# seanrjohnson/protein_gibbs_sampler

Hardware: AMD Instinct MI355X
Metric: sampled positions/sec (whole node), ESM-1b L=256 B=256 Gibbs (higher is better)
Workload: dtype bf16

## Files before the change

include/pgibbs.h:

```cpp
#ifndef PGIBBS_H
#define PGIBBS_H

#include <stdint.h>

#ifdef __cplusplus
extern "C" {
#endif

#define PG_OK 0
#define PG_ERR_INVALID 1
#define PG_ERR_HIP 2
#define PG_ERR_NO_DEVICE 3
#define PG_ERR_WEIGHTS 4
#define PG_ERR_UNSUPPORTED 5
#define PG_ERR_RANGE 6

const char* pg_version(void);
const char* pg_last_error(void);
int pg_device_count(void);

typedef struct pg_pyrandom pg_pyrandom;
pg_pyrandom* pg_pyrandom_create(void);
void pg_pyrandom_destroy(pg_pyrandom*);
int pg_pyrandom_seed(pg_pyrandom*, const uint32_t* key_words, int n_words);
// ... 104 lines not shown
                     int32_t* d_out);
typedef int (*pg_allgather_fn)(void* ctx, const void* send, void* recv, size_t n_int32);
int pg_dbg_gather_tokens_host(int rank, int world, const int32_t* local, int64_t rows, int width, const int64_t* counts,
                              int force_padded, pg_allgather_fn allgather, void* ctx, int32_t* out);
int pg_dbg_gather_plan(int rank, int world, int64_t rows, int width, const int64_t* counts, int force_padded, int64_t* out7,
                       int64_t* out_off_bytes);

int pg_prof_enable(pg_engine*, int on);
int pg_prof_reset(pg_engine*);
int pg_prof_get(pg_engine*, const char* kernel_class, double* total_ms, int64_t* launches);
int pg_prof_get_kernels(pg_engine*, const char* kernel_class, char* buf, int buf_bytes);

int pg_dbg_gemm(int device, int precision, const float* x, const float* w, const float* bias, float* out, int M, int N,
                int K, int epi);
int pg_dbg_gemm_bench(int device, int M, int N, int K, int epi, int variant, int iters, double* avg_ms);
int pg_dbg_gemm_plan(int M, int N, int K, int epi, int variant, int have_ws, int m_live, int n_cu, char* buf, int buf_bytes);
int pg_dbg_rowln_bench(int device, int M, int K, int iters, double* ms, double* max_diff);
int pg_dbg_qkv_attention_bench(int device, int B, int T, int H, int iters, double* ms, double* max_diff);
int pg_dbg_layernorm(int device, const float* x, const float* gamma, const float* beta, float* y, int M, int d,
                     float eps);
int pg_dbg_layernorm_operand(int device, int precision, const float* x, const float* gamma, const float* beta, float* y, int M,
                             int d, float eps);
int pg_dbg_attention(int device, int precision, const float* qkv, float* ctx, int B, int T, int H);
int pg_dbg_rope(int device, int precision, float* qkv_inout, int B, int T, int H);

int pg_dbg_msa_attention(int device, int which, const float* qkv, float* ctx, int B, int R, int C, int H, float scale);

#ifdef __cplusplus
}
#endif
#endif
```

protein_gibbs_sampler_amd/_lib.py:

```python
import ctypes
import math
import os
import sys
from ctypes import (POINTER, Structure, c_char_p, c_double, c_float, c_int, c_int32, c_int64, c_uint32, c_uint64,
                    c_void_p)

_HERE = os.path.dirname(os.path.abspath(__file__))
LIB_PATH = os.environ.get("PGIBBS_LIB_PATH") or os.path.join(_HERE, "lib", "libpgibbs.so")

PG_OK = 0
PG_ERR_INVALID, PG_ERR_HIP, PG_ERR_NO_DEVICE, PG_ERR_WEIGHTS, PG_ERR_UNSUPPORTED, PG_ERR_RANGE = 1, 2, 3, 4, 5, 6
PG_ARCH_ESM1B, PG_ARCH_MSA1B, PG_ARCH_ESM1, PG_ARCH_ESM2 = 1, 2, 3, 4
PG_COMM_ID_BYTES = 128
PG_PREC_BF16, PG_PREC_FP32, PG_PREC_F16 = 0, 1, 2
INT32_MAX = 2**31 - 1


class PgError(RuntimeError):
    def __init__(self, code, msg):
        super().__init__("pgibbs error %d: %s" % (code, msg))
        self.code = code
        self.msg = msg


# ... 63 lines not shown
    ("pg_mask_scatter_device", c_int, [c_void_p, c_void_p, c_int64, c_int, c_void_p, c_void_p, c_int64, c_int, c_int]),
    ("pg_sample_writeback_device", c_int, [c_void_p, c_void_p, c_int64, c_int, c_void_p, c_int, c_void_p, c_void_p, c_int64,
                                           c_int, POINTER(SampleParams), c_int, c_void_p]),
    ("pg_comm_unique_id", c_int, [c_void_p]),
    ("pg_comm_create", c_int, [c_int, c_int, c_void_p, c_int, POINTER(c_void_p)]),
    ("pg_comm_destroy", None, [c_void_p]),
    ("pg_comm_rank", c_int, [c_void_p]),
    ("pg_comm_world", c_int, [c_void_p]),
    ("pg_gather_tokens", c_int, [c_void_p, c_void_p, c_void_p, c_int64, c_int, POINTER(c_int64), c_void_p]),
    ("pg_dbg_gather_tokens_host", c_int, [c_int, c_int, c_void_p, c_int64, c_int, POINTER(c_int64), c_int, c_void_p, c_void_p, c_void_p]),
    ("pg_dbg_gather_plan", c_int, [c_int, c_int, c_int64, c_int, POINTER(c_int64), c_int, POINTER(c_int64), POINTER(c_int64)]),
    ("pg_prof_enable", c_int, [c_void_p, c_int]),
    ("pg_prof_reset", c_int, [c_void_p]),
    ("pg_prof_get", c_int, [c_void_p, c_char_p, POINTER(c_double), POINTER(c_int64)]),
    ("pg_prof_get_kernels", c_int, [c_void_p, c_char_p, c_char_p, c_int]),
    ("pg_dbg_gemm", c_int, [c_int, c_int, c_void_p, c_void_p, c_void_p, c_void_p, c_int, c_int, c_int, c_int]),
    ("pg_dbg_gemm_bench", c_int, [c_int, c_int, c_int, c_int, c_int, c_int, c_int, POINTER(c_double)]),
    ("pg_dbg_gemm_plan", c_int, [c_int, c_int, c_int, c_int, c_int, c_int, c_int, c_int, c_char_p, c_int]),
    ("pg_dbg_rowln_bench", c_int, [c_int, c_int, c_int, c_int, POINTER(c_double), POINTER(c_double)]),
    ("pg_dbg_qkv_attention_bench", c_int, [c_int, c_int, c_int, c_int, c_int, POINTER(c_double), POINTER(c_double)]),
    ("pg_dbg_layernorm", c_int, [c_int, c_void_p, c_void_p, c_void_p, c_void_p, c_int, c_int, c_float]),
    ("pg_dbg_layernorm_operand", c_int, [c_int, c_int, c_void_p, c_void_p, c_void_p, c_void_p, c_int, c_int, c_float]),
    ("pg_dbg_attention", c_int, [c_int, c_int, c_void_p, c_void_p, c_int, c_int, c_int]),
    ("pg_dbg_rope", c_int, [c_int, c_int, c_void_p, c_int, c_int, c_int]),
    ("pg_dbg_msa_attention", c_int, [c_int, c_int, c_void_p, c_void_p, c_int, c_int, c_int, c_int, c_float]),
]


def lib():
    global _lib
    if _lib is not None:
        return _lib
    if not os.path.exists(LIB_PATH):
        raise ImportError(
            "protein_gibbs_sampler_amd: the HIP library %s is missing. Build it with "
            "`python -c 'import __graft_entry__ as g; g.build()'` (or `make -C protein_gibbs_sampler_amd/csrc`). "
            "There is no CPU fallback." % LIB_PATH)
    if os.environ.get("PGIBBS_HIP_RUNTIME", "auto") != "system":
        try:
            import torch
        except ImportError:
            pass
    handle = ctypes.CDLL(LIB_PATH, mode=ctypes.RTLD_GLOBAL)
    for name, restype, argtypes in SIGNATURES:
        fn = getattr(handle, name)
        fn.restype = restype
# ... 34 lines not shown
```

protein_gibbs_sampler_amd/csrc/api.hip:

```cpp
#include <math.h>
#include <string.h>

#include <vector>

#include <algorithm>

#include "engine.h"
#include "gemm_epilogue.h"

namespace pg {
const char* last_error_cstr();
}
using namespace pg;

namespace {
struct DeviceGuard {
  int prev = -1;
  explicit DeviceGuard(int dev) {
    (void)hipGetDevice(&prev);
    if (dev >= 0 && dev != prev) (void)hipSetDevice(dev);
  }
  ~DeviceGuard() {
    if (prev >= 0) (void)hipSetDevice(prev);
  }
// ... 747 lines not shown
  Tmp t;
  float* dq = (float*)t.get((size_t)M * 3 * d * 4);
  if (precision == PG_PREC_FP32) {
    bf16_t* c3 = (bf16_t*)t.get((size_t)M * 3 * d * 2);
    if (!dq || !c3) return fail(PG_ERR_HIP, "hipMalloc failed");
    PG_HIP(hipMemcpy(dq, qkv, (size_t)M * 3 * d * 4, hipMemcpyHostToDevice));
    const SeqLayout chain = {1, T, 0, 1};
    if ((rc = launch_attention_f32(nullptr, dq, c3, d, B, T, H, 3 * d, 3 * d, d, 2 * d, chain))) return rc;
    return split3_rows_to_host(c3, ctx, M, d);
  }
  bf16_t* bq = (bf16_t*)t.get((size_t)M * 3 * d * 2);
  bf16_t* bc = (bf16_t*)t.get((size_t)M * d * 2);
  float* dc = (float*)t.get((size_t)M * d * 4);
  if (!dq || !bq || !bc || !dc) return fail(PG_ERR_HIP, "hipMalloc failed");
  PG_HIP(hipMemcpy(dq, qkv, (size_t)M * 3 * d * 4, hipMemcpyHostToDevice));
  if ((rc = OPS(launch_f32_to_bf16, nullptr, dq, bq, M * 3 * d, 1.f))) return rc;
  if ((rc = OPS(launch_attention_bf16, nullptr, bq, bc, B, T, H, 3 * d, d, d, 2 * d, nullptr, -1))) return rc;
  if ((rc = OPS(launch_bf16_to_f32, nullptr, bc, dc, M * d))) return rc;
  PG_HIP(hipDeviceSynchronize());
  PG_HIP(hipMemcpy(ctx, dc, (size_t)M * d * 4, hipMemcpyDeviceToHost));
  return PG_OK;
}

int pg_dbg_layernorm_operand(int device, int precision, const float* x, const float* gamma, const float* beta, float* y, int M, int d,
                             float eps) {
  if (precision != PG_PREC_BF16 && precision != PG_PREC_FP32 && precision != PG_PREC_F16) return fail(PG_ERR_INVALID, "unknown precision mode");
  if (!x || !gamma || !beta || !y || M < 1 || d < 32 || d % 32) return fail(PG_ERR_INVALID, "pg_dbg_layernorm_operand: bad argument");
  DeviceGuard g(-1);
  int rc = dbg_device(device);
  if (rc) return rc;
  const bool split = precision == PG_PREC_FP32;
  Tmp t;
  float* dx = (float*)t.get((size_t)M * d * 4);
  float* dg = (float*)t.get((size_t)d * 4);
  float* dbt = (float*)t.get((size_t)d * 4);
  float* dy = (float*)t.get((size_t)M * d * 4);
  bf16_t* h = (bf16_t*)t.get((size_t)M * d * 2 * (split ? 3 : 1));
  if (!dx || !dg || !dbt || !dy || !h) return fail(PG_ERR_HIP, "hipMalloc failed");
  PG_HIP(hipMemcpy(dx, x, (size_t)M * d * 4, hipMemcpyHostToDevice));
  PG_HIP(hipMemcpy(dg, gamma, (size_t)d * 4, hipMemcpyHostToDevice));
  PG_HIP(hipMemcpy(dbt, beta, (size_t)d * 4, hipMemcpyHostToDevice));
  if ((rc = OPS(launch_layernorm_bf16, nullptr, dx, dg, dbt, h, M, d, eps, split, 0, 0, true))) return rc;
  if (split) return split3_rows_to_host(h, y, M, d);
  if ((rc = OPS(launch_bf16_to_f32, nullptr, h, dy, (int64_t)M * d))) return rc;
  PG_HIP(hipDeviceSynchronize());
  PG_HIP(hipMemcpy(y, dy, (size_t)M * d * 4, hipMemcpyDeviceToHost));
// ... 75 lines not shown
```

protein_gibbs_sampler_amd/csrc/attention.hip:

```cpp
#include <stdlib.h>

#include "kernels.h"

PG_OPS_BEGIN

typedef __attribute__((ext_vector_type(8))) __bf16 bf16x8;
typedef __attribute__((ext_vector_type(4))) float f32x4;
typedef __attribute__((ext_vector_type(2))) float f32x2;

typedef short v4s __attribute__((ext_vector_type(4)));

#ifdef PG_ATT_PROF
__device__ unsigned long long* pg_att_prof;
#define PG_T(slot, i)                                                                                              \
  do {                                                                                                             \
    if ((slot) < 8 && (threadIdx.x & 63) == 0)                                                                     \
      pg_att_prof[(((size_t)blockIdx.x * 4 + (threadIdx.x >> 6)) * 8 + (slot)) * 8 + (i)] = __builtin_readcyclecounter(); \
  } while (0)
#else
#define PG_T(slot, i)
#endif

template <int MAXKB, bool PADMASK, bool BIASKV = false, bool SPLIT = false>
__global__ __launch_bounds__(256, (MAXKB <= 18 ? 2 : 1)) void attention_kernel(const bf16_t* __restrict__ qkv, bf16_t* __restrict__ ctx, int T,
                                                       int H, int ld_qkv_, int ld_ctx_, int k_off, int v_off,
                                                       SeqLayout sl, const int32_t* __restrict__ key_tok, int pad_idx,
                                                       const bf16_t* __restrict__ bias_kv, int split_from = 0, int split = 1) {
  __shared__ __attribute__((aligned(16))) char smem[2 * MAXKB * 16 * 128 + (PADMASK ? MAXKB * 16 : 0)];
  char* Ks = smem;
  char* Vs = smem + MAXKB * 16 * 128;
  char* padf = smem + 2 * MAXKB * 16 * 128;

  const int tid = threadIdx.x, lane = tid & 63, wave = tid >> 6;
  PG_T(7, 0);
  int pair = blockIdx.x, qb_first = wave, qb_step = 4;
  if (SPLIT && (int)blockIdx.x >= split_from) {
    const int u = blockIdx.x - split_from;
    pair = split_from + u / split;
    qb_first = u % split + split * wave;
    qb_step = 4 * split;
  }
  const int seq = pair / H, h = pair % H;
  const size_t row0 = (size_t)(seq / sl.inner_count) * sl.outer_rows + (size_t)(seq % sl.inner_count) * sl.inner_rows;
  const size_t ld_qkv = (size_t)ld_qkv_ * sl.row_step, ld_ctx = (size_t)ld_ctx_ * sl.row_step;
  const bf16_t* base = qkv + row0 * ld_qkv_ + h * 64;
  const int Tk = T + (BIASKV ? 1 : 0);
  constexpr int nkc = MAXKB / 2;
  constexpr int tpad = MAXKB * 16;

  {
    constexpr int NIT = (MAXKB * 16 * 8 + 255) / 256;
    uint4 kreg[NIT], vreg[NIT];
#pragma unroll
    for (int it = 0; it < NIT; ++it) {
      const int i = tid + it * 256;
      const int row = i >> 3, c = i & 7;
      kreg[it] = make_uint4(0, 0, 0, 0);
      vreg[it] = make_uint4(0, 0, 0, 0);
      if (i < tpad * 8 && row < T) {
        kreg[it] = *(const uint4*)(base + (size_t)row * ld_qkv + k_off + c * 8);
        vreg[it] = *(const uint4*)(base + (size_t)row * ld_qkv + v_off + c * 8);
      } else if (BIASKV && row == T) {
        kreg[it] = *(const uint4*)(bias_kv + h * 64 + c * 8);
        vreg[it] = *(const uint4*)(bias_kv + (H + h) * 64 + c * 8);
      }
    }
#pragma unroll
    for (int it = 0; it < NIT; ++it) {
      const int i = tid + it * 256;
      if (i < tpad * 8) {
// ... 3 lines not shown
      }
    }
  }
  if (PADMASK) {
    for (int key = tid; key < MAXKB * 16; key += 256)
      padf[key] = (key < T && key_tok[row0 + (size_t)key * sl.row_step] == pad_idx) ? 1 : 0;
  }
  PG_T(7, 1);
  __syncthreads();
  PG_T(7, 2);

  const int fr = lane & 15, fq = lane >> 4;
  const int nqb = (T + 15) >> 4;
  bf16x8 qf[2], qn[2];
  auto load_q = [&](int qb, bf16x8 (&dst)[2]) {
    int qrow = qb * 16 + fr;
    if (qrow >= T) qrow = T - 1;
#pragma unroll
    for (int kk = 0; kk < 2; ++kk) dst[kk] = *(const bf16x8*)(base + (size_t)qrow * ld_qkv + kk * 32 + fq * 8);
  };
  if (qb_first < nqb) load_q(qb_first, qf);
  for (int qb = qb_first; qb < nqb; qb += qb_step) {
    if (qb + qb_step < nqb) load_q(qb + qb_step, qn);
    PG_T(qb >> 2, 0);

    f32x4 st[MAXKB];
    {
      constexpr int CH = (MAXKB % 6 == 0) ? 6 : (MAXKB % 4 == 0 ? 4 : 2);
      bf16x8 kbuf[2][CH][2];
      auto load_chunk = [&](int ch, bf16x8 (&dst)[CH][2]) {
#pragma unroll
        for (int u = 0; u < CH; ++u) {
#if defined(PG_ATT_PROF) && PG_ATT_ABL == 1
          const int krow = (ch * CH + (u > 0 ? 0 : u)) * 16 + fr;
          if (u > 0) { dst[u][0] = dst[0][0]; dst[u][1] = dst[0][1]; continue; }
#else
          const int krow = (ch * CH + u) * 16 + fr;
#endif
#pragma unroll
          for (int kk = 0; kk < 2; ++kk) dst[u][kk] = *(const bf16x8*)(Ks + krow * 128 + (((kk * 4 + fq) ^ (krow & 7)) << 4));
        }
      };
      load_chunk(0, kbuf[0]);
#pragma unroll
      for (int ch = 0; ch < MAXKB / CH; ++ch) {
        if (ch + 1 < MAXKB / CH) load_chunk(ch + 1, kbuf[(ch + 1) & 1]);
        __builtin_amdgcn_sched_barrier(0);
#pragma unroll
        for (int u = 0; u < CH; ++u)
          st[ch * CH + u] = mfma_op16(kbuf[ch & 1][u][0], qf[0], (f32x4){0.f, 0.f, 0.f, 0.f});
#pragma unroll
        for (int u = 0; u < CH; ++u)
          st[ch * CH + u] = mfma_op16(kbuf[ch & 1][u][1], qf[1], st[ch * CH + u]);
        __builtin_amdgcn_sched_barrier(0);
      }
    }
    PG_T(qb >> 2, 1);
    float mx = -3.0e38f;
    int tl = Tk - fq * 4;
    asm volatile("" : "+v"(tl));
#pragma unroll
    for (int kb = MAXKB > 6 ? MAXKB - 6 : 0; kb < MAXKB; ++kb)
      if ((kb + 1) * 16 > Tk) {
#pragma unroll
        for (int r = 0; r < 4; ++r)
          if (kb * 16 + r >= tl) st[kb][r] = -3.0e38f;
      }
#pragma unroll
    for (int kb = 0; kb < MAXKB; ++kb)
#pragma unroll
      for (int r = 0; r < 4; ++r) mx = fmaxf(mx, st[kb][r]);
    if (PADMASK) {
      const float fill = sl.row_step == 1 ? -3.0e38f : -10000.0f;
      mx = -3.0e38f;
#pragma unroll
      for (int kb = 0; kb < MAXKB; ++kb) {
        const uint32_t f4 = *(const uint32_t*)(padf + kb * 16 + fq * 4);
#pragma unroll
        for (int r = 0; r < 4; ++r) {
          if ((f4 >> (8 * r)) & 0xffu) st[kb][r] = fill;
          mx = fmaxf(mx, st[kb][r]);
        }
      }
    }
    mx = rows4_max(mx);
    const f32x2 l2e = {1.44269504088896341f, 1.44269504088896341f};
    const float mneg1 = -mx * 1.44269504088896341f;
    const f32x2 mneg = {mneg1, mneg1};
    f32x2 sum2 = {0.f, 0.f};
#pragma unroll
    for (int kb = 0; kb < MAXKB; ++kb) {
      const f32x2 a = __builtin_elementwise_fma((f32x2){st[kb][0], st[kb][1]}, l2e, mneg);
      const f32x2 b = __builtin_elementwise_fma((f32x2){st[kb][2], st[kb][3]}, l2e, mneg);
      const f32x2 ea = {__builtin_amdgcn_exp2f(a[0]), __builtin_amdgcn_exp2f(a[1])};
      const f32x2 eb = {__builtin_amdgcn_exp2f(b[0]), __builtin_amdgcn_exp2f(b[1])};
      st[kb] = (f32x4){ea[0], ea[1], eb[0], eb[1]};
      sum2 += ea;
      sum2 += eb;
    }
    float sum = sum2[0] + sum2[1];
    sum = rows4_sum(sum);
    const float inv = 1.0f / sum;
    PG_T(qb >> 2, 2);

    f32x4 o[4];
#pragma unroll
    for (int db = 0; db < 4; ++db) o[db] = (f32x4){0.f, 0.f, 0.f, 0.f};
    {
      union VF { bf16x8 v; uint2 h[2]; };
      VF vbuf[3][4];
      auto load_v = [&](int c, VF (&dst)[4]) {
#pragma unroll
        for (int db = 0; db < 4; ++db) {
#if defined(PG_ATT_PROF) && PG_ATT_ABL == 2
          if (db > 0) { dst[db] = dst[0]; continue; }
#endif
#pragma unroll
          for (int hh = 0; hh < 2; ++hh) {
            const int krow = (2 * c + hh) * 16 + fq * 4 + (fr >> 2);
            const int dcol = db * 16 + (fr & 3) * 4;
            const char* a = Vs + krow * 128 + (((dcol >> 3) ^ (krow & 7)) << 4) + ((dcol >> 2) & 1) * 8;
            const v4s t = __builtin_amdgcn_ds_read_tr16_b64_v4i16((v4s __attribute__((address_space(3)))*)(
                (__attribute__((address_space(3))) char*)a));
            dst[db].h[hh] = __builtin_bit_cast(uint2, t);
          }
        }
      };
      load_v(0, vbuf[0]);
      if (nkc > 1) load_v(1, vbuf[1]);
#pragma unroll
      for (int c = 0; c < nkc; ++c) {
        if (c + 2 < nkc) load_v(c + 2, vbuf[(c + 2) % 3]);
        union { bf16x8 v; uint32_t u[4]; } pf;
        const f32x4 lo = st[2 * c], hi = st[2 * c + 1];
        pf.u[0] = pack_op2(lo[0], lo[1]);
        pf.u[1] = pack_op2(lo[2], lo[3]);
        pf.u[2] = pack_op2(hi[0], hi[1]);
        pf.u[3] = pack_op2(hi[2], hi[3]);
        __builtin_amdgcn_sched_barrier(0);
#pragma unroll
        for (int db = 0; db < 4; ++db) o[db] = mfma_op16(vbuf[c % 3][db].v, pf.v, o[db]);
        __builtin_amdgcn_sched_barrier(0);
      }
    }
    PG_T(qb >> 2, 3);
    const int q = qb * 16 + fr;
    if (q < T) {
      bf16_t* dst = ctx + row0 * ld_ctx_ + (size_t)q * ld_ctx + h * 64 + fq * 4;
#pragma unroll
      for (int db = 0; db < 4; ++db) {
        uint2 p;
        p.x = pack_op2(o[db][0] * inv, o[db][1] * inv);
        p.y = pack_op2(o[db][2] * inv, o[db][3] * inv);
        *(uint2*)(dst + db * 16) = p;
      }
    }
    qf[0] = qn[0];
    qf[1] = qn[1];
    PG_T(qb >> 2, 4);
  }
  PG_T(7, 3);
}

template <int MAXKB, int OCC, bool PADMASK, bool BIASKV>
__global__ __launch_bounds__(256, OCC) void attention_long_kernel(const bf16_t* __restrict__ qkv, bf16_t* __restrict__ ctx, int T,
                                                               int H, int ld_qkv_, int ld_ctx_, int k_off, int v_off,
                                                               SeqLayout sl, int n_qchunk, const int32_t* __restrict__ key_tok_,
                                                               int pad_idx, const bf16_t* __restrict__ bias_kv_) {
  const int32_t* __restrict__ key_tok = PADMASK ? key_tok_ : nullptr;
  const bf16_t* __restrict__ bias_kv = BIASKV ? bias_kv_ : nullptr;
  constexpr int tpad = MAXKB * 16, nkc = MAXKB / 2;
  __shared__ __attribute__((aligned(16))) char smem[2 * tpad * 128 + (PADMASK ? tpad : 0)];
  char* Ks = smem;
  char* Vs = smem + tpad * 128;
  char* padf = smem + 2 * tpad * 128;
  const int tid = threadIdx.x, lane = tid & 63, wave = tid >> 6;
  const int qc = blockIdx.x % n_qchunk, sh = blockIdx.x / n_qchunk;
  const int seq = sh / H, h = sh % H;
  const size_t row0 = (size_t)(seq / sl.inner_count) * sl.outer_rows + (size_t)(seq % sl.inner_count) * sl.inner_rows;
  const size_t ld_qkv = (size_t)ld_qkv_ * sl.row_step, ld_ctx = (size_t)ld_ctx_ * sl.row_step;
  const bf16_t* base = qkv + row0 * ld_qkv_ + h * 64;
  const int fr = lane & 15, fq = lane >> 4;
  const int q0 = qc * 64 + wave * 16;
  const bool active = q0 < T;
// ... 120 lines not shown
      }
    }
  }
  const int q = q0 + fr;
  if (active && q < T) {
    const float inv = 1.0f / l;
    bf16_t* dst = ctx + row0 * ld_ctx_ + (size_t)q * ld_ctx + h * 64 + fq * 4;
#pragma unroll
    for (int db = 0; db < 4; ++db) {
      uint2 p;
      p.x = pack_op2(o[db][0] * inv, o[db][1] * inv);
      p.y = pack_op2(o[db][2] * inv, o[db][3] * inv);
      *(uint2*)(dst + db * 16) = p;
    }
  }
}

int launch_attention_bf16(hipStream_t s, const bf16_t* qkv, bf16_t* ctx, int B, int T, int H, int ld_qkv, int ld_ctx,
                          int k_off, int v_off, const int32_t* key_tok, int pad_idx, const bf16_t* bias_kv) {
  SeqLayout sl = {1, T, 0, 1};
  return launch_attention_seq_bf16(s, qkv, ctx, B, T, H, ld_qkv, ld_ctx, k_off, v_off, sl, key_tok, pad_idx, bias_kv);
}

int launch_attention_seq_bf16(hipStream_t s, const bf16_t* qkv, bf16_t* ctx, int64_t n_seq, int T, int H, int ld_qkv,
                              int ld_ctx, int k_off, int v_off, SeqLayout sl, const int32_t* key_tok, int pad_idx,
                              const bf16_t* bias_kv) {
  if (n_seq == 0) return 0;
  if (n_seq * H > 0x7fffffff) return fail(1, "attention: too many sequences");
  dim3 grid((unsigned)(n_seq * H)), block(256);
  static const int split_on = env_int("PGIBBS_ATTN_SPLIT", 1);
  const int n_cu = device_cu_count();
  int split_from = 0, split = 1;
  if (split_on && !key_tok && !bias_kv && sl.row_step == 1 && T >= 64 && T <= 576) {
    const int kb = (((T + 15) / 16) + 1) & ~1;
    const long pairs = n_seq * H, slots = (long)n_cu * (kb <= 20 ? 2 : 1);
    const long rem = pairs % slots;
    const int nqb = (T + 15) / 16;
    int sp = rem ? (int)(slots / rem) : 1;
    if (sp > 4) sp = 4;
    if (sp > nqb / 4) sp = nqb / 4;
    if (sp >= 2) {
      split = sp;
      split_from = (int)(pairs - rem);
      grid = dim3((unsigned)(split_from + rem * sp));
    }
  }
#define PG_ATT_SPLIT_LAUNCH(KB) hipLaunchKernelGGL((attention_kernel<KB, false, false, true>), grid, block, 0, s, qkv, ctx, T, H, ld_qkv, ld_ctx, k_off, v_off, sl, key_tok, pad_idx, bias_kv, split_from, split)
#define PG_ATT(KB)                                                                                             \
  else if (Tk <= KB * 16) {                                                                                    \
    if (bias_kv && key_tok) hipLaunchKernelGGL((attention_kernel<KB, true, true>), grid, block, 0, s, qkv, ctx, T, H, ld_qkv, ld_ctx, k_off, v_off, sl, key_tok, pad_idx, bias_kv); \
    else if (bias_kv) hipLaunchKernelGGL((attention_kernel<KB, false, true>), grid, block, 0, s, qkv, ctx, T, H, ld_qkv, ld_ctx, k_off, v_off, sl, key_tok, pad_idx, bias_kv); \
    else if (key_tok) hipLaunchKernelGGL((attention_kernel<KB, true>), grid, block, 0, s, qkv, ctx, T, H, ld_qkv, ld_ctx, k_off, v_off, sl, key_tok, pad_idx, bias_kv); \
    else if (split > 1) PG_ATT_SPLIT_LAUNCH(KB);                                                               \
    else hipLaunchKernelGGL((attention_kernel<KB, false>), grid, block, 0, s, qkv, ctx, T, H, ld_qkv, ld_ctx, k_off, v_off, sl, key_tok, pad_idx, bias_kv); \
  }
  const int Tk = T + (bias_kv ? 1 : 0);
  static const int fine_ladder = env_int("PGIBBS_ATTN_LADDER", 1);
  if (T <= 0) return fail(1, "attention: empty sequence");
#define PG_ATT_PLAIN(KB)                                                                                       \
  else if (fine_ladder && !bias_kv && Tk <= KB * 16) {                                                         \
    if (key_tok) hipLaunchKernelGGL((attention_kernel<KB, true>), grid, block, 0, s, qkv, ctx, T, H, ld_qkv, ld_ctx, k_off, v_off, sl, key_tok, pad_idx, bias_kv); \
    else if (split > 1) PG_ATT_SPLIT_LAUNCH(KB);                                                               \
    else hipLaunchKernelGGL((attention_kernel<KB, false>), grid, block, 0, s, qkv, ctx, T, H, ld_qkv, ld_ctx, k_off, v_off, sl, key_tok, pad_idx, bias_kv); \
  }
  PG_ATT(2) PG_ATT(4) PG_ATT_PLAIN(6) PG_ATT(8) PG_ATT_PLAIN(10) PG_ATT(12) PG_ATT_PLAIN(14) PG_ATT_PLAIN(16) PG_ATT(18)
  PG_ATT_PLAIN(20) PG_ATT_PLAIN(22) PG_ATT(24) PG_ATT_PLAIN(26) PG_ATT_PLAIN(28) PG_ATT(30) PG_ATT_PLAIN(32) PG_ATT_PLAIN(34) PG_ATT(36)
#undef PG_ATT_PLAIN
#undef PG_ATT
#undef PG_ATT_SPLIT_LAUNCH
  else {
    const int n_qchunk = (T + 63) / 64;
    if (n_seq * H * n_qchunk > 0x7fffffff) return fail(1, "attention: too many sequences");
    const dim3 g((unsigned)(n_seq * H * n_qchunk));
#define PG_ATT_LONG(P, B) hipLaunchKernelGGL((attention_long_kernel<18, 2, P, B>), g, block, 0, s, qkv, ctx, T, H, ld_qkv, ld_ctx, k_off, v_off, sl, n_qchunk, key_tok, pad_idx, bias_kv)
    if (key_tok && bias_kv) PG_ATT_LONG(true, true);
    else if (key_tok) PG_ATT_LONG(true, false);
    else if (bias_kv) PG_ATT_LONG(false, true);
    else PG_ATT_LONG(false, false);
#undef PG_ATT_LONG
  }
  PG_HIP(hipGetLastError());
  return 0;
}

PG_OPS_END
```

protein_gibbs_sampler_amd/csrc/kernels_ops.inc:

```
int launch_gemm_bf16(hipStream_t s, const bf16_t* X, const bf16_t* W, const float* bias, void* out, int M, int N, int K,
                     int ldx, int ldw, int ldo, int epi, float* ws = nullptr, size_t ws_bytes = 0, int m_live = 0);
int gemm_splitk_splits(int K);
size_t gemm_splitk_ws_bytes(int M, int N, int K);
int launch_gemm_bf16_variant(hipStream_t s, const bf16_t* X, const bf16_t* W, const float* bias, void* out, int M, int N,
                             int K, int ldx, int ldw, int ldo, int epi, int variant, float* ws = nullptr, size_t ws_bytes = 0,
                             int m_live = 0);

bool gemm_ln_skinny_ok(int M, int N, int K);
int launch_gemm_ln_skinny(hipStream_t s, const float* X, int ldx, const float* gamma, const float* beta, float eps, const bf16_t* W,
                          const float* bias, void* out, int M, int N, int K, int ldw, int ldo, int epi);
bool chain_trunk_ok(int M, int d_model, int d_ffn, int n_heads);
size_t chain_trunk_sync_bytes();
size_t chain_trunk_part_bytes(int M, int d_model);
int launch_chain_trunk(hipStream_t s, const PgChainTrunkArgs& a, int M, int d_model);
int launch_gemm_big(hipStream_t s, const bf16_t* X, const bf16_t* W, const float* bias, void* out, int M, int N, int K, int ldx,
                    int ldw, int ldo, int epi, int m_live = 0);
bool gemm_ladder_has(int epi, int h);
int launch_gemm_ladder(hipStream_t s, const bf16_t* X, const bf16_t* W, const float* bias, void* out, int m_live, int m_rows, int h,
                       int N, int K, int ldx, int ldw, int ldo, int epi);
bool gemm_rowln_ok(int m_rows, int N, int K);
int launch_gemm_rowln(hipStream_t s, const bf16_t* A, const bf16_t* W, const float* bias, float* x, const float* gamma,
                      const float* beta, bf16_t* h, int m_live, int m_rows, int K, int lda, int ldw, float eps, int colmajor_R = 0,
                      int colmajor_C = 0, int abl = 0);
void gemm_plan_text(int M, int N, int K, int epi, int variant, bool have_ws, int m_live, int n_cu, std::string* text);
void gemm_big_geometry(int M, int N, int K, int* m_main_panels, int* tail_rows);
int launch_gemm_w16(hipStream_t s, const bf16_t* X, const bf16_t* W, const float* bias, void* out, int M, int N, int K, int ldx,
                    int ldw, int ldo, int epi, int abl = 0, int tail_rows = 0);
int launch_gemm_split3(hipStream_t s, const bf16_t* X3, const bf16_t* W3, const float* bias, void* out, int M, int N, int K, int ldo,
                       int epi);
bool gemm_split3_fused(int M, int N, int K, int epi);
int launch_gemm_split3_w16(hipStream_t s, const bf16_t* X3, const bf16_t* W3, const float* bias, void* out, int M, int N, int K,
                           int ldo, int epi);

int launch_attention_bf16(hipStream_t s, const bf16_t* qkv, bf16_t* ctx, int B, int T, int H, int ld_qkv, int ld_ctx,
                          int k_off, int v_off, const int32_t* key_tok = nullptr, int pad_idx = -1, const bf16_t* bias_kv = nullptr);
int launch_attention_seq_bf16(hipStream_t s, const bf16_t* qkv, bf16_t* ctx, int64_t n_seq, int T, int H, int ld_qkv,
                              int ld_ctx, int k_off, int v_off, SeqLayout sl, const int32_t* key_tok = nullptr,
                              int pad_idx = -1, const bf16_t* bias_kv = nullptr);
size_t msa_row_split_scratch_bytes(int B, int R, int C, int H, int order_bh);
int launch_msa_row_attention_bf16(hipStream_t s, const bf16_t* qkv, bf16_t* ctx, int B, int R, int C, int H, int ld_qkv,
                                  int ld_ctx, int k_off, int v_off, float scale, float* partial = nullptr,
                                  size_t partial_bytes = 0, int order_bh = 0);

int launch_embed_ln(hipStream_t s, const int32_t* tokens, const float* embed, const float* pos, const float* msa_pos,
                    const float* gamma, const float* beta, float* x, int64_t n_tok, int T, int d, int pad_idx,
                    int mask_idx, int token_dropout, int rows_per_msa, float eps,
                    const float* gamma2 = nullptr, const float* beta2 = nullptr, bf16_t* h2 = nullptr,
                    float embed_scale = 1.0f);
int launch_rope(hipStream_t s, void* qkv, bool f32, const float* table, int table_rows, int64_t M, int T, int H, int ld);
int launch_layernorm_bf16(hipStream_t s, const float* x, const float* gamma, const float* beta, bf16_t* h, int64_t M,
                          int d, float eps, bool split3 = false,
                          int colmajor_R = 0, int colmajor_C = 0,
                          bool split3_dup = true);
bool colattn_ok(int R, int d_model, int n_heads);
int launch_gemm_colattn(hipStream_t s, const bf16_t* X, const bf16_t* W, const float* bias, bf16_t* ctx, int B, int R, int C, int H,
                        int d, int ld_ctx);
int launch_headmajor_qkv(hipStream_t s, const bf16_t* w, const float* b, bf16_t* w2, float* b2, int H, int K);
int launch_layernorm_f32(hipStream_t s, const float* x, const float* gamma, const float* beta, float* y, int64_t M, int d,
                         float eps);
int launch_gather_ln_bf16(hipStream_t s, const float* x, const int32_t* idx, const int32_t* row_map, int P, int width,
                          const float* gamma, const float* beta, bf16_t* h, int64_t n_sel, int d, float eps,
// ... 19 lines not shown
```

Measured before the change: 72600.

## Add persistent attention kernel with double-buffered K/V DMA and ticketed q-blocks

```diff
diff --git a/include/pgibbs.h b/include/pgibbs.h
--- a/include/pgibbs.h
+++ b/include/pgibbs.h
@@ -150,6 +150,8 @@
 int pg_dbg_layernorm_operand(int device, int precision, const float* x, const float* gamma, const float* beta, float* y, int M,
                              int d, float eps);
 int pg_dbg_attention(int device, int precision, const float* qkv, float* ctx, int B, int T, int H);
+int pg_dbg_attention_forms(int device, int precision, const uint16_t* qkv, uint16_t* ctx_plain, uint16_t* ctx_persistent, int B, int T,
+                           int H, int iters, double* ms);
 int pg_dbg_rope(int device, int precision, float* qkv_inout, int B, int T, int H);
 
 int pg_dbg_msa_attention(int device, int which, const float* qkv, float* ctx, int B, int R, int C, int H, float scale);
diff --git a/protein_gibbs_sampler_amd/_lib.py b/protein_gibbs_sampler_amd/_lib.py
--- a/protein_gibbs_sampler_amd/_lib.py
+++ b/protein_gibbs_sampler_amd/_lib.py
@@ -109,6 +109,7 @@
     ("pg_dbg_layernorm", c_int, [c_int, c_void_p, c_void_p, c_void_p, c_void_p, c_int, c_int, c_float]),
     ("pg_dbg_layernorm_operand", c_int, [c_int, c_int, c_void_p, c_void_p, c_void_p, c_void_p, c_int, c_int, c_float]),
     ("pg_dbg_attention", c_int, [c_int, c_int, c_void_p, c_void_p, c_int, c_int, c_int]),
+    ("pg_dbg_attention_forms", c_int, [c_int, c_int, c_void_p, c_void_p, c_void_p, c_int, c_int, c_int, c_int, POINTER(c_double)]),
     ("pg_dbg_rope", c_int, [c_int, c_int, c_void_p, c_int, c_int, c_int]),
     ("pg_dbg_msa_attention", c_int, [c_int, c_int, c_void_p, c_void_p, c_int, c_int, c_int, c_int, c_float]),
 ]
diff --git a/protein_gibbs_sampler_amd/csrc/api.hip b/protein_gibbs_sampler_amd/csrc/api.hip
--- a/protein_gibbs_sampler_amd/csrc/api.hip
+++ b/protein_gibbs_sampler_amd/csrc/api.hip
@@ -793,6 +793,47 @@
   return PG_OK;
 }
 
+int pg_dbg_attention_forms(int device, int precision, const uint16_t* qkv, uint16_t* ctx_plain, uint16_t* ctx_persistent, int B, int T,
+                           int H, int iters, double* ms) {
+  if (precision != PG_PREC_BF16 && precision != PG_PREC_F16) return fail(PG_ERR_INVALID, "pg_dbg_attention_forms: bf16 or fp16 operands");
+  if (!qkv || !ctx_plain || !ctx_persistent || B < 1 || T < 1 || H < 1 || (iters > 0 && !ms))
+    return fail(PG_ERR_INVALID, "pg_dbg_attention_forms: bad argument");
+  DeviceGuard g(-1);
+  int rc = dbg_device(device);
+  if (rc) return rc;
+  const int d = H * 64;
+  const size_t M = (size_t)B * T;
+  Tmp t;
+  bf16_t* bq = (bf16_t*)t.get(M * 3 * d * 2);
+  bf16_t* bc = (bf16_t*)t.get(M * d * 2);
+  if (!bq || !bc) return fail(PG_ERR_HIP, "hipMalloc failed");
+  PG_HIP(hipMemcpy(bq, qkv, M * 3 * d * 2, hipMemcpyHostToDevice));
+  const SeqLayout chain = {1, T, 0, 1};
+  hipEvent_t e0, e1;
+  PG_HIP(hipEventCreate(&e0));
+  PG_HIP(hipEventCreate(&e1));
+  for (int form = 1; form <= 2 && !rc; ++form) {
+    PG_HIP(hipMemset(bc, 0xff, M * d * 2));
+    rc = OPS(launch_attention_seq_bf16, nullptr, bq, bc, B, T, H, 3 * d, d, d, 2 * d, chain, nullptr, -1, nullptr, form);
+    if (rc) break;
+    PG_HIP(hipDeviceSynchronize());
+    PG_HIP(hipMemcpy(form == 1 ? ctx_plain : ctx_persistent, bc, M * d * 2, hipMemcpyDeviceToHost));
+    if (iters > 0) {
+      PG_HIP(hipEventRecord(e0, nullptr));
+      for (int it = 0; it < iters && !rc; ++it)
+        rc = OPS(launch_attention_seq_bf16, nullptr, bq, bc, B, T, H, 3 * d, d, d, 2 * d, chain, nullptr, -1, nullptr, form);
+      PG_HIP(hipEventRecord(e1, nullptr));
+      PG_HIP(hipEventSynchronize(e1));
+      float el = 0.f;
+      PG_HIP(hipEventElapsedTime(&el, e0, e1));
+      ms[form - 1] = el / iters;
+    }
+  }
+  (void)hipEventDestroy(e0);
+  (void)hipEventDestroy(e1);
+  return rc;
+}
+
 int pg_dbg_layernorm_operand(int device, int precision, const float* x, const float* gamma, const float* beta, float* y, int M, int d,
                              float eps) {
   if (precision != PG_PREC_BF16 && precision != PG_PREC_FP32 && precision != PG_PREC_F16) return fail(PG_ERR_INVALID, "unknown precision mode");
diff --git a/protein_gibbs_sampler_amd/csrc/attention.hip b/protein_gibbs_sampler_amd/csrc/attention.hip
--- a/protein_gibbs_sampler_amd/csrc/attention.hip
+++ b/protein_gibbs_sampler_amd/csrc/attention.hip
@@ -1,11 +1,10 @@
 #include <stdlib.h>
 
+#include "gemm_epilogue.h"
 #include "kernels.h"
 
 PG_OPS_BEGIN
 
-typedef __attribute__((ext_vector_type(8))) __bf16 bf16x8;
-typedef __attribute__((ext_vector_type(4))) float f32x4;
 typedef __attribute__((ext_vector_type(2))) float f32x2;
 
 typedef short v4s __attribute__((ext_vector_type(4)));
@@ -21,6 +20,146 @@
 #define PG_T(slot, i)
 #endif
 
+template <int MAXKB, bool PADMASK>
+__device__ __forceinline__ void attention_qblock(const char* Ks, const char* Vs, const char* padf, const bf16x8 (&qf)[2], int qb, int T,
+                                                 int Tk, float pad_fill, bf16_t* ctx_head, size_t ld_ctx, int fr, int fq, int slot) {
+  constexpr int nkc = MAXKB / 2;
+  PG_T(slot, 0);
+
+  f32x4 st[MAXKB];
+  {
+    constexpr int CH = (MAXKB % 6 == 0) ? 6 : (MAXKB % 4 == 0 ? 4 : 2);
+    bf16x8 kbuf[2][CH][2];
+    auto load_chunk = [&](int ch, bf16x8 (&dst)[CH][2]) {
+#pragma unroll
+      for (int u = 0; u < CH; ++u) {
+#if defined(PG_ATT_PROF) && PG_ATT_ABL == 1
+        const int krow = (ch * CH + (u > 0 ? 0 : u)) * 16 + fr;
+        if (u > 0) { dst[u][0] = dst[0][0]; dst[u][1] = dst[0][1]; continue; }
+#else
+        const int krow = (ch * CH + u) * 16 + fr;
+#endif
+#pragma unroll
+        for (int kk = 0; kk < 2; ++kk) dst[u][kk] = *(const bf16x8*)(Ks + krow * 128 + (((kk * 4 + fq) ^ (krow & 7)) << 4));
+      }
+    };
+    load_chunk(0, kbuf[0]);
+#pragma unroll
+    for (int ch = 0; ch < MAXKB / CH; ++ch) {
+      if (ch + 1 < MAXKB / CH) load_chunk(ch + 1, kbuf[(ch + 1) & 1]);
+      __builtin_amdgcn_sched_barrier(0);
+#pragma unroll
+      for (int u = 0; u < CH; ++u)
+        st[ch * CH + u] = mfma_op16(kbuf[ch & 1][u][0], qf[0], (f32x4){0.f, 0.f, 0.f, 0.f});
+#pragma unroll
+      for (int u = 0; u < CH; ++u)
+        st[ch * CH + u] = mfma_op16(kbuf[ch & 1][u][1], qf[1], st[ch * CH + u]);
+      __builtin_amdgcn_sched_barrier(0);
+    }
+  }
+  PG_T(slot, 1);
+  float mx = -3.0e38f;
+  int tl = Tk - fq * 4;
+  asm volatile("" : "+v"(tl));
+#pragma unroll
+  for (int kb = MAXKB > 6 ? MAXKB - 6 : 0; kb < MAXKB; ++kb)
+    if ((kb + 1) * 16 > Tk) {
+#pragma unroll
+      for (int r = 0; r < 4; ++r)
+        if (kb * 16 + r >= tl) st[kb][r] = -3.0e38f;
+    }
+#pragma unroll
+  for (int kb = 0; kb < MAXKB; ++kb)
+#pragma unroll
+    for (int r = 0; r < 4; ++r) mx = fmaxf(mx, st[kb][r]);
+  if (PADMASK) {
+    const float fill = pad_fill;
+    mx = -3.0e38f;
+#pragma unroll
+    for (int kb = 0; kb < MAXKB; ++kb) {
+      const uint32_t f4 = *(const uint32_t*)(padf + kb * 16 + fq * 4);
+#pragma unroll
+      for (int r = 0; r < 4; ++r) {
+        if ((f4 >> (8 * r)) & 0xffu) st[kb][r] = fill;
+        mx = fmaxf(mx, st[kb][r]);
+      }
+    }
+  }
+  mx = rows4_max(mx);
+  const f32x2 l2e = {1.44269504088896341f, 1.44269504088896341f};
+  const float mneg1 = -mx * 1.44269504088896341f;
+  const f32x2 mneg = {mneg1, mneg1};
+  f32x2 sum2 = {0.f, 0.f};
+#pragma unroll
+  for (int kb = 0; kb < MAXKB; ++kb) {
+    const f32x2 a = __builtin_elementwise_fma((f32x2){st[kb][0], st[kb][1]}, l2e, mneg);
+    const f32x2 b = __builtin_elementwise_fma((f32x2){st[kb][2], st[kb][3]}, l2e, mneg);
+    const f32x2 ea = {__builtin_amdgcn_exp2f(a[0]), __builtin_amdgcn_exp2f(a[1])};
+    const f32x2 eb = {__builtin_amdgcn_exp2f(b[0]), __builtin_amdgcn_exp2f(b[1])};
+    st[kb] = (f32x4){ea[0], ea[1], eb[0], eb[1]};
+    sum2 += ea;
+    sum2 += eb;
+  }
+  float sum = sum2[0] + sum2[1];
+  sum = rows4_sum(sum);
+  const float inv = 1.0f / sum;
+  PG_T(slot, 2);
+
+  f32x4 o[4];
+#pragma unroll
+  for (int db = 0; db < 4; ++db) o[db] = (f32x4){0.f, 0.f, 0.f, 0.f};
+  {
+    union VF { bf16x8 v; uint2 h[2]; };
+    VF vbuf[3][4];
+    auto load_v = [&](int c, VF (&dst)[4]) {
+#pragma unroll
+      for (int db = 0; db < 4; ++db) {
+#if defined(PG_ATT_PROF) && PG_ATT_ABL == 2
+        if (db > 0) { dst[db] = dst[0]; continue; }
+#endif
+#pragma unroll
+        for (int hh = 0; hh < 2; ++hh) {
+          const int krow = (2 * c + hh) * 16 + fq * 4 + (fr >> 2);
+          const int dcol = db * 16 + (fr & 3) * 4;
+          const char* a = Vs + krow * 128 + (((dcol >> 3) ^ (krow & 7)) << 4) + ((dcol >> 2) & 1) * 8;
+          const v4s t = __builtin_amdgcn_ds_read_tr16_b64_v4i16((v4s __attribute__((address_space(3)))*)(
+              (__attribute__((address_space(3))) char*)a));
+          dst[db].h[hh] = __builtin_bit_cast(uint2, t);
+        }
+      }
+    };
+    load_v(0, vbuf[0]);
+    if (nkc > 1) load_v(1, vbuf[1]);
+#pragma unroll
+    for (int c = 0; c < nkc; ++c) {
+      if (c + 2 < nkc) load_v(c + 2, vbuf[(c + 2) % 3]);
+      union { bf16x8 v; uint32_t u[4]; } pf;
+      const f32x4 lo = st[2 * c], hi = st[2 * c + 1];
+      pf.u[0] = pack_op2(lo[0], lo[1]);
+      pf.u[1] = pack_op2(lo[2], lo[3]);
+      pf.u[2] = pack_op2(hi[0], hi[1]);
+      pf.u[3] = pack_op2(hi[2], hi[3]);
+      __builtin_amdgcn_sched_barrier(0);
+#pragma unroll
+      for (int db = 0; db < 4; ++db) o[db] = mfma_op16(vbuf[c % 3][db].v, pf.v, o[db]);
+      __builtin_amdgcn_sched_barrier(0);
+    }
+  }
+  PG_T(slot, 3);
+  const int q = qb * 16 + fr;
+  if (q < T) {
+    bf16_t* dst = ctx_head + (size_t)q * ld_ctx + fq * 4;
+#pragma unroll
+    for (int db = 0; db < 4; ++db) {
+      uint2 p;
+      p.x = pack_op2(o[db][0] * inv, o[db][1] * inv);
+      p.y = pack_op2(o[db][2] * inv, o[db][3] * inv);
+      *(uint2*)(dst + db * 16) = p;
+    }
+  }
+  PG_T(slot, 4);
+}
+
 template <int MAXKB, bool PADMASK, bool BIASKV = false, bool SPLIT = false>
 __global__ __launch_bounds__(256, (MAXKB <= 18 ? 2 : 1)) void attention_kernel(const bf16_t* __restrict__ qkv, bf16_t* __restrict__ ctx, int T,
                                                        int H, int ld_qkv_, int ld_ctx_, int k_off, int v_off,
@@ -45,7 +184,6 @@
   const size_t ld_qkv = (size_t)ld_qkv_ * sl.row_step, ld_ctx = (size_t)ld_ctx_ * sl.row_step;
   const bf16_t* base = qkv + row0 * ld_qkv_ + h * 64;
   const int Tk = T + (BIASKV ? 1 : 0);
-  constexpr int nkc = MAXKB / 2;
   constexpr int tpad = MAXKB * 16;
 
   {
@@ -95,144 +233,103 @@
   if (qb_first < nqb) load_q(qb_first, qf);
   for (int qb = qb_first; qb < nqb; qb += qb_step) {
     if (qb + qb_step < nqb) load_q(qb + qb_step, qn);
-    PG_T(qb >> 2, 0);
-
-    f32x4 st[MAXKB];
-    {
-      constexpr int CH = (MAXKB % 6 == 0) ? 6 : (MAXKB % 4 == 0 ? 4 : 2);
-      bf16x8 kbuf[2][CH][2];
-      auto load_chunk = [&](int ch, bf16x8 (&dst)[CH][2]) {
-#pragma unroll
-        for (int u = 0; u < CH; ++u) {
-#if defined(PG_ATT_PROF) && PG_ATT_ABL == 1
-          const int krow = (ch * CH + (u > 0 ? 0 : u)) * 16 + fr;
-          if (u > 0) { dst[u][0] = dst[0][0]; dst[u][1] = dst[0][1]; continue; }
-#else
-          const int krow = (ch * CH + u) * 16 + fr;
-#endif
-#pragma unroll
-          for (int kk = 0; kk < 2; ++kk) dst[u][kk] = *(const bf16x8*)(Ks + krow * 128 + (((kk * 4 + fq) ^ (krow & 7)) << 4));
-        }
-      };
-      load_chunk(0, kbuf[0]);
-#pragma unroll
-      for (int ch = 0; ch < MAXKB / CH; ++ch) {
-        if (ch + 1 < MAXKB / CH) load_chunk(ch + 1, kbuf[(ch + 1) & 1]);
-        __builtin_amdgcn_sched_barrier(0);
-#pragma unroll
-        for (int u = 0; u < CH; ++u)
-          st[ch * CH + u] = mfma_op16(kbuf[ch & 1][u][0], qf[0], (f32x4){0.f, 0.f, 0.f, 0.f});
-#pragma unroll
-        for (int u = 0; u < CH; ++u)
-          st[ch * CH + u] = mfma_op16(kbuf[ch & 1][u][1], qf[1], st[ch * CH + u]);
-        __builtin_amdgcn_sched_barrier(0);
-      }
-    }
-    PG_T(qb >> 2, 1);
-    float mx = -3.0e38f;
-    int tl = Tk - fq * 4;
-    asm volatile("" : "+v"(tl));
-#pragma unroll
-    for (int kb = MAXKB > 6 ? MAXKB - 6 : 0; kb < MAXKB; ++kb)
-      if ((kb + 1) * 16 > Tk) {
-#pragma unroll
-        for (int r = 0; r < 4; ++r)
-          if (kb * 16 + r >= tl) st[kb][r] = -3.0e38f;
-      }
-#pragma unroll
-    for (int kb = 0; kb < MAXKB; ++kb)
-#pragma unroll
-      for (int r = 0; r < 4; ++r) mx = fmaxf(mx, st[kb][r]);
-    if (PADMASK) {
-      const float fill = sl.row_step == 1 ? -3.0e38f : -10000.0f;
-      mx = -3.0e38f;
-#pragma unroll
-      for (int kb = 0; kb < MAXKB; ++kb) {
-        const uint32_t f4 = *(const uint32_t*)(padf + kb * 16 + fq * 4);
-#pragma unroll
-        for (int r = 0; r < 4; ++r) {
-          if ((f4 >> (8 * r)) & 0xffu) st[kb][r] = fill;
-          mx = fmaxf(mx, st[kb][r]);
-        }
-      }
-    }
-    mx = rows4_max(mx);
-    const f32x2 l2e = {1.44269504088896341f, 1.44269504088896341f};
-    const float mneg1 = -mx * 1.44269504088896341f;
-    const f32x2 mneg = {mneg1, mneg1};
-    f32x2 sum2 = {0.f, 0.f};
-#pragma unroll
-    for (int kb = 0; kb < MAXKB; ++kb) {
-      const f32x2 a = __builtin_elementwise_fma((f32x2){st[kb][0], st[kb][1]}, l2e, mneg);
-      const f32x2 b = __builtin_elementwise_fma((f32x2){st[kb][2], st[kb][3]}, l2e, mneg);
-      const f32x2 ea = {__builtin_amdgcn_exp2f(a[0]), __builtin_amdgcn_exp2f(a[1])};
-      const f32x2 eb = {__builtin_amdgcn_exp2f(b[0]), __builtin_amdgcn_exp2f(b[1])};
-      st[kb] = (f32x4){ea[0], ea[1], eb[0], eb[1]};
-      sum2 += ea;
-      sum2 += eb;
-    }
-    float sum = sum2[0] + sum2[1];
-    sum = rows4_sum(sum);
-    const float inv = 1.0f / sum;
-    PG_T(qb >> 2, 2);
-
-    f32x4 o[4];
-#pragma unroll
-    for (int db = 0; db < 4; ++db) o[db] = (f32x4){0.f, 0.f, 0.f, 0.f};
-    {
-      union VF { bf16x8 v; uint2 h[2]; };
-      VF vbuf[3][4];
-      auto load_v = [&](int c, VF (&dst)[4]) {
-#pragma unroll
-        for (int db = 0; db < 4; ++db) {
-#if defined(PG_ATT_PROF) && PG_ATT_ABL == 2
-          if (db > 0) { dst[db] = dst[0]; continue; }
-#endif
-#pragma unroll
-          for (int hh = 0; hh < 2; ++hh) {
-            const int krow = (2 * c + hh) * 16 + fq * 4 + (fr >> 2);
-            const int dcol = db * 16 + (fr & 3) * 4;
-            const char* a = Vs + krow * 128 + (((dcol >> 3) ^ (krow & 7)) << 4) + ((dcol >> 2) & 1) * 8;
-            const v4s t = __builtin_amdgcn_ds_read_tr16_b64_v4i16((v4s __attribute__((address_space(3)))*)(
-                (__attribute__((address_space(3))) char*)a));
-            dst[db].h[hh] = __builtin_bit_cast(uint2, t);
-          }
-        }
-      };
-      load_v(0, vbuf[0]);
-      if (nkc > 1) load_v(1, vbuf[1]);
-#pragma unroll
-      for (int c = 0; c < nkc; ++c) {
-        if (c + 2 < nkc) load_v(c + 2, vbuf[(c + 2) % 3]);
-        union { bf16x8 v; uint32_t u[4]; } pf;
-        const f32x4 lo = st[2 * c], hi = st[2 * c + 1];
-        pf.u[0] = pack_op2(lo[0], lo[1]);
-        pf.u[1] = pack_op2(lo[2], lo[3]);
-        pf.u[2] = pack_op2(hi[0], hi[1]);
-        pf.u[3] = pack_op2(hi[2], hi[3]);
-        __builtin_amdgcn_sched_barrier(0);
-#pragma unroll
-        for (int db = 0; db < 4; ++db) o[db] = mfma_op16(vbuf[c % 3][db].v, pf.v, o[db]);
-        __builtin_amdgcn_sched_barrier(0);
-      }
-    }
-    PG_T(qb >> 2, 3);
-    const int q = qb * 16 + fr;
-    if (q < T) {
-      bf16_t* dst = ctx + row0 * ld_ctx_ + (size_t)q * ld_ctx + h * 64 + fq * 4;
-#pragma unroll
-      for (int db = 0; db < 4; ++db) {
-        uint2 p;
-        p.x = pack_op2(o[db][0] * inv, o[db][1] * inv);
-        p.y = pack_op2(o[db][2] * inv, o[db][3] * inv);
-        *(uint2*)(dst + db * 16) = p;
-      }
-    }
+    attention_qblock<MAXKB, PADMASK>(Ks, Vs, padf, qf, qb, T, Tk, sl.row_step == 1 ? -3.0e38f : -10000.0f,
+                                     ctx + row0 * ld_ctx_ + h * 64, ld_ctx, fr, fq, qb >> 2);
     qf[0] = qn[0];
     qf[1] = qn[1];
-    PG_T(qb >> 2, 4);
   }
   PG_T(7, 3);
+}
+
+template <int MAXKB>
+__global__ __launch_bounds__(512, 1) void attention_persistent_kernel(const bf16_t* __restrict__ qkv, bf16_t* __restrict__ ctx, int T,
+                                                                      int H, int ld_qkv_, int ld_ctx_, int k_off, int v_off,
+                                                                      SeqLayout sl, int n_pairs) {
+  constexpr int HALF = MAXKB * 16 * 128, BUF = 2 * HALF;
+  constexpr int NPIECE = MAXKB * 2;
+  __shared__ __attribute__((aligned(16))) char smem[2 * BUF];
+  __shared__ int ctl[8];
+  auto ctl_load = [&](int i) { return __hip_atomic_load(&ctl[i], __ATOMIC_RELAXED, __HIP_MEMORY_SCOPE_WORKGROUP); };
+  auto ctl_store = [&](int i, int v) { __hip_atomic_store(&ctl[i], v, __ATOMIC_RELAXED, __HIP_MEMORY_SCOPE_WORKGROUP); };
+  auto ctl_add = [&](int i) { return __hip_atomic_fetch_add(&ctl[i], 1, __ATOMIC_RELAXED, __HIP_MEMORY_SCOPE_WORKGROUP); };
+
+  const int tid = threadIdx.x, lane = tid & 63;
+  const int wave = __builtin_amdgcn_readfirstlane(tid >> 6);
+  const int fr = lane & 15, fq = lane >> 4;
+  const int nqb = (T + 15) >> 4;
+  const int np = (n_pairs - (int)blockIdx.x + (int)gridDim.x - 1) / (int)gridDim.x;
+  const int total = np * nqb;
+  const size_t ld_qkv = (size_t)ld_qkv_ * sl.row_step, ld_ctx = (size_t)ld_ctx_ * sl.row_step;
+  auto pair_row0 = [&](int j, int& h) -> size_t {
+    const int pair = blockIdx.x + j * gridDim.x, seq = pair / H;
+    h = pair - seq * H;
+    return (size_t)(seq / sl.inner_count) * sl.outer_rows + (size_t)(seq % sl.inner_count) * sl.inner_rows;
+  };
+  const int dma_voff = (int)(((lane >> 3) * ld_qkv + (((lane & 7) ^ (lane >> 3)) << 3)) * 2);
+  const int piece_bytes = (int)(8 * ld_qkv * 2);
+  const unsigned tile_bytes = (unsigned)(((size_t)(T - 1) * ld_qkv + 64) * 2);
+  auto dma_pair = [&](int j, int b, int first, int step) {
+    int h;
+    const size_t row0 = pair_row0(j, h);
+    const bf16_t* src = qkv + row0 * ld_qkv_ + h * 64;
+    const rsrc_t rk = __builtin_amdgcn_make_buffer_rsrc((void*)(src + k_off), 0, tile_bytes, 0x00020000);
+    const rsrc_t rv = __builtin_amdgcn_make_buffer_rsrc((void*)(src + v_off), 0, tile_bytes, 0x00020000);
+    char* dst = smem + b * BUF;
+    for (int p = first; p < NPIECE; p += step) {
+      __builtin_amdgcn_raw_ptr_buffer_load_lds(rk, PG_LDS_PTR(dst + p * 1024), 16, dma_voff, p * piece_bytes, 0, 0);
+      __builtin_amdgcn_raw_ptr_buffer_load_lds(rv, PG_LDS_PTR(dst + HALF + p * 1024), 16, dma_voff, p * piece_bytes, 0, 0);
+    }
+  };
+  auto take_ticket = [&]() -> int {
+    int t = 0;
+    if (lane == 0) t = ctl_add(0);
+    return __builtin_amdgcn_readfirstlane(t);
+  };
+  bf16x8 qf[2], qn[2];
+  auto load_q = [&](int t, bf16x8 (&dst)[2]) {
+    const int j = t / nqb, qb = t - j * nqb;
+    int h;
+    const size_t row0 = pair_row0(j, h);
+    int qrow = qb * 16 + fr;
+    if (qrow >= T) qrow = T - 1;
+#pragma unroll
+    for (int kk = 0; kk < 2; ++kk) dst[kk] = *(const bf16x8*)(qkv + row0 * ld_qkv_ + h * 64 + (size_t)qrow * ld_qkv + kk * 32 + fq * 8);
+  };
+
+  if (tid < 8) ctl_store(tid, tid == 3 ? 1 : (tid == 4 ? 2 : 0));
+  dma_pair(0, 0, wave, 8);
+  if (np > 1) dma_pair(1, 1, wave, 8);
+  asm volatile("s_waitcnt vmcnt(0)" ::: "memory");
+  __syncthreads();
+
+  int nxt = take_ticket();
+  if (nxt < total) load_q(nxt, qn);
+  while (nxt < total) {
+    const int cur = nxt;
+    qf[0] = qn[0];
+    qf[1] = qn[1];
+    asm volatile("" : "+v"(qf[0]), "+v"(qf[1]));
+    nxt = take_ticket();
+    if (nxt < total) load_q(nxt, qn);
+    const int j = cur / nqb, qb = cur - j * nqb, b = j & 1;
+    while (ctl_load(3 + b) != j + 1) __builtin_amdgcn_s_sleep(1);
+    asm volatile("" ::: "memory");
+    int h;
+    const size_t row0 = pair_row0(j, h);
+    const char* Ks = smem + b * BUF;
+    attention_qblock<MAXKB, false>(Ks, Ks + HALF, nullptr, qf, qb, T, T, 0.f, ctx + row0 * ld_ctx_ + h * 64, ld_ctx, fr, fq, 8);
+    asm volatile("s_waitcnt lgkmcnt(0)" ::: "memory");
+    int fin = 0;
+    if (lane == 0) fin = ctl_add(1 + b);
+    if (__builtin_amdgcn_readfirstlane(fin) == nqb - 1) {
+      ctl_store(1 + b, 0);
+      if (j + 2 < np) {
+        dma_pair(j + 2, b, 0, 1);
+        asm volatile("s_waitcnt vmcnt(0)" ::: "memory");
+        ctl_store(3 + b, j + 3);
+      }
+    }
+  }
 }
 
 template <int MAXKB, int OCC, bool PADMASK, bool BIASKV>
@@ -399,14 +496,35 @@
   return launch_attention_seq_bf16(s, qkv, ctx, B, T, H, ld_qkv, ld_ctx, k_off, v_off, sl, key_tok, pad_idx, bias_kv);
 }
 
+constexpr int kPersistentMinPairsPerCu = 3;
+bool attention_persistent_eligible(int T, SeqLayout sl, const int32_t* key_tok, const bf16_t* bias_kv) {
+  return !key_tok && !bias_kv && sl.row_step == 1 && T > 192 && T <= 288;
+}
+
 int launch_attention_seq_bf16(hipStream_t s, const bf16_t* qkv, bf16_t* ctx, int64_t n_seq, int T, int H, int ld_qkv,
                               int ld_ctx, int k_off, int v_off, SeqLayout sl, const int32_t* key_tok, int pad_idx,
-                              const bf16_t* bias_kv) {
+                              const bf16_t* bias_kv, int form) {
   if (n_seq == 0) return 0;
   if (n_seq * H > 0x7fffffff) return fail(1, "attention: too many sequences");
+  if (T <= 0) return fail(1, "attention: empty sequence");
+  const int n_cu = device_cu_count();
+  const bool can_persist = attention_persistent_eligible(T, sl, key_tok, bias_kv);
+#ifdef PG_ATT_PROF
+  if (form == 0) form = 1;
+#endif
+  if (form == 2 && !can_persist) return fail(1, "attention: the persistent form does not serve this launch");
+  if (form == 2 || (form == 0 && can_persist && n_seq * H >= (int64_t)kPersistentMinPairsPerCu * n_cu)) {
+    const int n_pairs = (int)(n_seq * H);
+    const dim3 g((unsigned)(n_pairs < n_cu ? n_pairs : n_cu)), b(512);
+#define PG_ATT_PERSIST(KB) else if (T <= KB * 16) hipLaunchKernelGGL((attention_persistent_kernel<KB>), g, b, 0, s, qkv, ctx, T, H, ld_qkv, ld_ctx, k_off, v_off, sl, n_pairs)
+    if (false) {}
+    PG_ATT_PERSIST(14); PG_ATT_PERSIST(16); PG_ATT_PERSIST(18);
+#undef PG_ATT_PERSIST
+    PG_HIP(hipGetLastError());
+    return 0;
+  }
   dim3 grid((unsigned)(n_seq * H)), block(256);
   static const int split_on = env_int("PGIBBS_ATTN_SPLIT", 1);
-  const int n_cu = device_cu_count();
   int split_from = 0, split = 1;
   if (split_on && !key_tok && !bias_kv && sl.row_step == 1 && T >= 64 && T <= 576) {
     const int kb = (((T + 15) / 16) + 1) & ~1;
@@ -433,13 +551,13 @@
   }
   const int Tk = T + (bias_kv ? 1 : 0);
   static const int fine_ladder = env_int("PGIBBS_ATTN_LADDER", 1);
-  if (T <= 0) return fail(1, "attention: empty sequence");
 #define PG_ATT_PLAIN(KB)                                                                                       \
   else if (fine_ladder && !bias_kv && Tk <= KB * 16) {                                                         \
     if (key_tok) hipLaunchKernelGGL((attention_kernel<KB, true>), grid, block, 0, s, qkv, ctx, T, H, ld_qkv, ld_ctx, k_off, v_off, sl, key_tok, pad_idx, bias_kv); \
     else if (split > 1) PG_ATT_SPLIT_LAUNCH(KB);                                                               \
     else hipLaunchKernelGGL((attention_kernel<KB, false>), grid, block, 0, s, qkv, ctx, T, H, ld_qkv, ld_ctx, k_off, v_off, sl, key_tok, pad_idx, bias_kv); \
   }
+  if (false) {}
   PG_ATT(2) PG_ATT(4) PG_ATT_PLAIN(6) PG_ATT(8) PG_ATT_PLAIN(10) PG_ATT(12) PG_ATT_PLAIN(14) PG_ATT_PLAIN(16) PG_ATT(18)
   PG_ATT_PLAIN(20) PG_ATT_PLAIN(22) PG_ATT(24) PG_ATT_PLAIN(26) PG_ATT_PLAIN(28) PG_ATT(30) PG_ATT_PLAIN(32) PG_ATT_PLAIN(34) PG_ATT(36)
 #undef PG_ATT_PLAIN
diff --git a/protein_gibbs_sampler_amd/csrc/kernels_ops.inc b/protein_gibbs_sampler_amd/csrc/kernels_ops.inc
--- a/protein_gibbs_sampler_amd/csrc/kernels_ops.inc
+++ b/protein_gibbs_sampler_amd/csrc/kernels_ops.inc
@@ -36,7 +36,7 @@
                           int k_off, int v_off, const int32_t* key_tok = nullptr, int pad_idx = -1, const bf16_t* bias_kv = nullptr);
 int launch_attention_seq_bf16(hipStream_t s, const bf16_t* qkv, bf16_t* ctx, int64_t n_seq, int T, int H, int ld_qkv,
                               int ld_ctx, int k_off, int v_off, SeqLayout sl, const int32_t* key_tok = nullptr,
-                              int pad_idx = -1, const bf16_t* bias_kv = nullptr);
+                              int pad_idx = -1, const bf16_t* bias_kv = nullptr, int form = 0);
 size_t msa_row_split_scratch_bytes(int B, int R, int C, int H, int order_bh);
 int launch_msa_row_attention_bf16(hipStream_t s, const bf16_t* qkv, bf16_t* ctx, int B, int R, int C, int H, int ld_qkv,
                                   int ld_ctx, int k_off, int v_off, float scale, float* partial = nullptr,
```

Measured after the change: 72970, median of 6. About the same (+0.5%).
